# Aakash1312/Fluid-Simulation

Hardware: AMD Instinct MI355X
Metric: simulated substeps/sec (higher is better)
Workload: dtype f64

## Files before the change

### fluid-simulation_amd/csrc/common.h

```cpp
#pragma once
#include <hip/hip_runtime.h>
#include <stdint.h>

namespace fl {

constexpr uint8_t F_SOLID = 1;
constexpr uint8_t F_FLUID = 2;
constexpr int F_CNT_SHIFT = 2;

struct Grid {
    int N;
    int lo;
    int hi;
    int nx, ny, nz;
    int ox, oy, oz;
    __host__ __device__ inline size_t idx(int ix, int iy, int iz) const
    {
        return ((size_t)ix * ny + (size_t)iy) * nz + (size_t)iz;
    }
    __host__ __device__ inline size_t cells() const { return (size_t)nx * ny * nz; }
    __host__ __device__ inline long sx() const { return (long)ny * nz; }
    __host__ __device__ inline int cx0() const { return lo + ox; }
    __host__ __device__ inline int cy0() const { return lo + oy; }
    __host__ __device__ inline int cz0() const { return lo + oz; }
// ... 58 lines not shown
    int max_cell;
    int n_drop;
    int n_tl_mg, n_tl_sq;
    int n_rows, n_l1_old;
    int n_tl_int, n_tl_bnd;
    int n_l1_gal, n_drop_fail;
    unsigned long long max_speed_bits;
    double dt;
    double err_num;
    double err_den;
};

constexpr size_t STATE_PS_OFF = 256;
constexpr int MAX_PARTIALS = 8192;

__device__ __forceinline__ double spline(double x)
{
    if (x < 0) x *= -1.0;
    if (x < 0.5) return 1.5 * (4.0 * x * x * x - 4.0 * x * x + 2.0 / 3.0);
    if (x < 1.0) return 1.5 * ((-8.0 * (x * x * x) / 6.0) + 4.0 * x * x - 4.0 * x + 4.0 / 3.0);
    return 0;
}

__device__ __forceinline__ double spline_at(double p, int c, int d)
{
    double x = p - (double)c;
    if (d == 1) return spline(x);
    if (x < 0) x *= -1.0;
    if (x < 1.0) return 1.5 * ((-8.0 * (x * x * x) / 6.0) + 4.0 * x * x - 4.0 * x + 4.0 / 3.0);
    return 0;
}

template <typename T>
__device__ __forceinline__ T wave_sum(T v)
{
#pragma unroll
    for (int o = 32; o > 0; o >>= 1) v += __shfl_down(v, o, 64);
    return v;
}
template <typename T>
__device__ __forceinline__ T wave_max(T v)
{
#pragma unroll
    for (int o = 32; o > 0; o >>= 1) {
// ... 106 lines not shown
    uint32_t* pid;
    __host__ __device__ inline Particles shifted(long o) const
    {
        Particles q = *this;
        q.px += o; q.py += o; q.pz += o; q.vx += o; q.vy += o; q.vz += o; q.pid += o;
        return q;
    }
};
constexpr uint32_t PID_DEAD = 0xFFFFFFFFu;

void launch_bin_count(hipStream_t st, Grid g, long n, Particles p, int* key, int* slot, int* cell_count, int* part, StepState* ss);
void launch_bin_scatter(hipStream_t st, long n, const int* key, const int* slot, const int* cell_start, const uint32_t* pid, int* order,
                         uint32_t* spid);
void launch_bin_rank(hipStream_t st, long n_pos, long pos0, const int* key, const int* cell_start, const int* order, const uint32_t* spid,
                     int* order2);
void launch_reorder(hipStream_t st, long n, const int* order, Particles src, Particles dst, double* w = nullptr, long wstride = 0);
void launch_weights(hipStream_t st, long n, Particles p, double* w, long stride);
void launch_axpby_box(hipStream_t st, Grid g, Box box, double a, const double* x, double b, const double* y, double* out, const PcgState* gate = nullptr);
long p2g_max_items(Box box);
size_t p2g_part_doubles(Box box);
constexpr int P2G_PILED = 256;
void launch_p2g(hipStream_t st, Grid g, Box box, Particles p, const double* pw, long wstride, const int* cell_start, const uint8_t* flags,
                double* part, int* items, float* container, double* u, double* v, double* w, double* ub, double* vb, double* wb, int2* crowd_list = nullptr,
                Particles park = Particles{});
void launch_p2g_tiles(hipStream_t st, Grid g, Box box, Particles p, const double* pw, long wstride, const int* cell_start, const uint8_t* flags,
                      float* container, double* u, double* v, double* w, double* ub, double* vb, double* wb);
void launch_g2p_tiled(hipStream_t st, Grid g, Box pb, Particles p, const int* cell_start, const double* dcx, const double* dcy, const double* dcz,
                      const double* pcx, const double* pcy, const double* pcz, double blend, StepState* ss);
void launch_g2p(hipStream_t st, Grid g, long n, Particles p, const double* dcx, const double* dcy, const double* dcz, const double* pcx,
                const double* pcy, const double* pcz, double blend, StepState* ss);
void launch_advect(hipStream_t st, Grid g, long n, Particles p, const uint8_t* flags, double max_dt, double dx, StepState* ss);
void launch_advect_bin(hipStream_t st, Grid g, long n, Particles p, const uint8_t* flags, double max_dt, double dx, StepState* ss, int* key,
                       int* slot, int* cell_count, int* part);
void launch_pack_particles(hipStream_t st, long n, Particles p, double* pos_aos, double* vel_aos);
void launch_unpack_records(hipStream_t st, long n, const double* rec, Particles p, long off);
void launch_pack_records(hipStream_t st, long n, Particles p, long off, double* rec);
void launch_unpack_ids(hipStream_t st, long n, const double* pos, const double* vel, const uint32_t* ids, Particles p);
void launch_pack_ids(hipStream_t st, long n, Particles p, long off, double* pos, double* vel, uint32_t* ids);
void launch_unpack_particles(hipStream_t st, long n, const double* pos_aos, const double* vel_aos, Particles p);

// ... 222 lines not shown
```

### fluid-simulation_amd/csrc/fluid_api.hip

```cpp
#include "sim.h"
#include <algorithm>

using namespace fl;

static thread_local std::string g_err;
int fluid_fail(int code, const std::string& msg)
{
    g_err = msg;
    return code;
}
#define fail fluid_fail

Box fl::clip_dilate(const Box& b, int d, const Grid& g)
{
    Box r;
    r.x0 = b.x0 - d < 0 ? 0 : b.x0 - d;
    r.y0 = b.y0 - d < 0 ? 0 : b.y0 - d;
    r.z0 = b.z0 - d < 0 ? 0 : b.z0 - d;
    r.x1 = b.x1 + d > g.nx - 1 ? g.nx - 1 : b.x1 + d;
    r.y1 = b.y1 + d > g.ny - 1 ? g.ny - 1 : b.y1 + d;
    r.z1 = b.z1 + d > g.nz - 1 ? g.nz - 1 : b.z1 + d;
    return r;
}

// ... 33 lines not shown
        }
        p.e0.clear();
        p.e1.clear();
        p.pc.clear();
    }
}


static void free_particles(fluid_sim* s)
{
    for (Particles* p : {&s->pa, &s->pb}) {
        hipFree(p->px); hipFree(p->py); hipFree(p->pz); hipFree(p->vx); hipFree(p->vy); hipFree(p->vz); hipFree(p->pid);
        *p = Particles{};
    }
    hipFree(s->key); hipFree(s->slot); hipFree(s->order); hipFree(s->order2); hipFree(s->spid); hipFree(s->stage_pos); hipFree(s->stage_vel);
    s->order2 = nullptr; s->spid = nullptr; hipFree(s->pw);
    s->pw = nullptr;
    s->key = s->slot = s->order = nullptr;
    s->binned = false;
    s->stage_pos = s->stage_vel = nullptr;
    s->cap = 0;
}

int fl::alloc_particles(fluid_sim* s, long n)
{
    if (n <= s->cap) return FLUID_OK;
    n = (n + 1) & ~1L;
    free_particles(s);
    for (Particles* p : {&s->pa, &s->pb}) {
        HIPCHK(dalloc(&p->px, n)); HIPCHK(dalloc(&p->py, n)); HIPCHK(dalloc(&p->pz, n));
        HIPCHK(dalloc(&p->vx, n)); HIPCHK(dalloc(&p->vy, n)); HIPCHK(dalloc(&p->vz, n));
        HIPCHK(dalloc(&p->pid, n));
    }
    HIPCHK(dalloc(&s->key, n)); HIPCHK(dalloc(&s->slot, n)); HIPCHK(dalloc(&s->order, n)); HIPCHK(dalloc(&s->order2, n)); HIPCHK(dalloc(&s->spid, n));
    HIPCHK(dalloc(&s->stage_pos, 3 * n)); HIPCHK(dalloc(&s->stage_vel, 3 * n));
    HIPCHK(dalloc(&s->pw, 9 * n));
    HIPCHK(hipDeviceSynchronize());
    s->cap = n;
    return FLUID_OK;
}

int fl::grow_particles(fluid_sim* s, long need)
{
    if (need <= s->cap) return FLUID_OK;
    HIPCHK(hipStreamSynchronize(s->st));
    const long keep = s->p_off + s->np;
    Particles old = s->pa;
    s->pa = Particles{};
    const long ncap = ((need + need / 2) + 1) & ~1L;
    Particles nw{};
    HIPCHK(dalloc(&nw.px, ncap)); HIPCHK(dalloc(&nw.py, ncap)); HIPCHK(dalloc(&nw.pz, ncap));
// ... 2 lines not shown
    if (keep > 0) {
        HIPCHK(hipMemcpy(nw.px, old.px, keep * 8, hipMemcpyDeviceToDevice)); HIPCHK(hipMemcpy(nw.py, old.py, keep * 8, hipMemcpyDeviceToDevice));
        HIPCHK(hipMemcpy(nw.pz, old.pz, keep * 8, hipMemcpyDeviceToDevice)); HIPCHK(hipMemcpy(nw.vx, old.vx, keep * 8, hipMemcpyDeviceToDevice));
        HIPCHK(hipMemcpy(nw.vy, old.vy, keep * 8, hipMemcpyDeviceToDevice)); HIPCHK(hipMemcpy(nw.vz, old.vz, keep * 8, hipMemcpyDeviceToDevice));
        HIPCHK(hipMemcpy(nw.pid, old.pid, keep * 4, hipMemcpyDeviceToDevice));
    }
    hipFree(old.px); hipFree(old.py); hipFree(old.pz); hipFree(old.vx); hipFree(old.vy); hipFree(old.vz); hipFree(old.pid);
    free_particles(s);
    s->pa = nw;
    Particles* p = &s->pb;
    HIPCHK(dalloc(&p->px, ncap)); HIPCHK(dalloc(&p->py, ncap)); HIPCHK(dalloc(&p->pz, ncap));
    HIPCHK(dalloc(&p->vx, ncap)); HIPCHK(dalloc(&p->vy, ncap)); HIPCHK(dalloc(&p->vz, ncap));
    HIPCHK(dalloc(&p->pid, ncap));
    HIPCHK(dalloc(&s->key, ncap)); HIPCHK(dalloc(&s->slot, ncap)); HIPCHK(dalloc(&s->order, ncap)); HIPCHK(dalloc(&s->order2, ncap)); HIPCHK(dalloc(&s->spid, ncap));
    HIPCHK(dalloc(&s->stage_pos, 3 * ncap)); HIPCHK(dalloc(&s->stage_vel, 3 * ncap));
    HIPCHK(dalloc(&s->pw, 9 * ncap));
    HIPCHK(hipDeviceSynchronize());
    s->cap = ncap;
    return FLUID_OK;
}

extern "C" {

const char* fluid_last_error(void) { return g_err.c_str(); }
const char* fluid_version(void) { return "libfluid_hip 0.1 gfx950"; }

int fluid_default_params(fluid_params_t* p)
{
    if (!p) return fail(FLUID_ERR_ARG, "null params");
    memset(p, 0, sizeof(*p));
    p->n = 121;
// ... 340 lines not shown
    s->sort_hint = true;
    s->n_out = s->h_ss->n_out;
    s->max_cell = s->h_ss->max_cell;
    const StepState& h = *s->h_ss;
    if (h.bbox_max[0] < 0) {
        s->Pb = Box{0, 0, 0, -1, -1, -1};
    } else {
        s->Pb = Box{h.bbox_min[0], h.bbox_min[1], h.bbox_min[2], h.bbox_max[0], h.bbox_max[1], h.bbox_max[2]};
    }
    if (!box_empty(s->Pb)) {
        s->Rb = clip_dilate(s->Pb, 1, g);
        s->Sb = clip_dilate(s->Pb, 2, g);
    } else {
        s->Rb = s->Sb = s->Pb;
    }
    launch_reorder(s->st, s->np, s->order2, s->pa.shifted(s->p_off), s->pb, s->pw, s->cap);
    HIPCHK(hipGetLastError());
    std::swap(s->pa, s->pb);
    s->p_off = 0;
    prof_end(s, FLUID_PROF_SORT, tok);
    s->sorted = true;
    return FLUID_OK;
}

int fl::run_p2g(fluid_sim* s, const Box& box)
{
    const long ref_cells = s->p2g_ref_cells > 0 ? s->p2g_ref_cells : s->Rb.cells();
    const bool airy = s->last_num_active > 0 && (double)s->last_num_active < 0.3 * (double)ref_cells;
    const bool huge = (size_t)12 * sizeof(double) * (size_t)box.cells() > ((size_t)16 << 30);
    const bool piled = s->max_cell > P2G_PILED || airy;
    if (s->p2g_force ? s->p2g_force == 2 : huge) {
        s->stats.paths |= FLUID_PATH_P2G_TILES;
        launch_p2g_tiles(s->st, s->g, box, s->pa, s->pw, s->cap, s->cell_start, s->flags, s->container, s->u, s->v, s->w, s->ub, s->vb, s->wb);
        return FLUID_OK;
    }
    const bool crowd = s->p2g_force ? s->p2g_force == 3 : piled;
    if (crowd) {
        s->stats.paths |= FLUID_PATH_P2G_CROWD;
        const size_t nl = (size_t)s->cap / 16 + 64;
        if (nl > s->p2g_crowd_cap) {
            if (s->p2g_crowd) { HIPCHK(hipStreamSynchronize(s->st)); hipFree(s->p2g_crowd); s->p2g_crowd = nullptr; }
            HIPCHK(hipMalloc((void**)&s->p2g_crowd, nl * sizeof(int2)));
            s->p2g_crowd_cap = nl;
        }
    }
    const size_t need = p2g_part_doubles(box);
    if (need > s->p2g_part_cap) {
        if (s->p2g_part) { HIPCHK(hipStreamSynchronize(s->st)); hipFree(s->p2g_part); s->p2g_part = nullptr; }
        HIPCHK(hipMalloc((void**)&s->p2g_part, (need + need / 4) * sizeof(double)));
        s->p2g_part_cap = need + need / 4;
    }
    const size_t ni = 4 + 4 * (size_t)p2g_max_items(box);
    if (ni > s->p2g_items_cap) {
        if (s->p2g_items) { HIPCHK(hipStreamSynchronize(s->st)); hipFree(s->p2g_items); s->p2g_items = nullptr; }
        HIPCHK(hipMalloc((void**)&s->p2g_items, (ni + ni / 4) * sizeof(int)));
        HIPCHK(hipMemsetAsync(s->p2g_items, 0, 4 * sizeof(int), s->st));
        s->p2g_items_cap = ni + ni / 4;
    }
    launch_p2g(s->st, s->g, box, s->pa, s->pw, s->cap, s->cell_start, s->flags, s->p2g_part, s->p2g_items, s->container, s->u, s->v, s->w, s->ub,
               s->vb, s->wb, crowd ? s->p2g_crowd : nullptr, s->pb);
    return FLUID_OK;
}

static int phase_p2g(fluid_sim* s)
{
    HIPCHK(hipSetDevice(s->prm.device));
    int rc = phase_sort(s);
    if (rc) return rc;
    rc = clear_dirty(s);
    if (rc) return rc;
    memset(&s->stats, 0, sizeof(s->stats));
    s->stats.dt_in = s->dt;
    s->stats.dt_out = s->dt;
    for (int a = 0; a < 3; ++a) {
// ... 1019 lines not shown
```

### fluid-simulation_amd/csrc/fluid_dist.hip

```cpp
#include "sim.h"
#include "dist_kernels.h"

using namespace fl;
#define fail fluid_fail
int cuts_from_hist(int n, const int64_t* hist, int P, int32_t* cuts);

#define COMMCHK(expr)                                                                              \
    do {                                                                                           \
        if ((expr) != 0) return fail(FLUID_ERR_HIP, std::string("comm callback failed: ") + #expr); \
    } while (0)

namespace {

constexpr int HALO_W = 4;

struct IBox {
    int lo[3], hi[3];
};
inline bool ib_empty(const IBox& b) { return b.hi[0] <= b.lo[0] || b.hi[1] <= b.lo[1] || b.hi[2] <= b.lo[2]; }
inline IBox ib_isect(const IBox& a, const IBox& b)
{
    IBox r;
    for (int k = 0; k < 3; ++k) { r.lo[k] = std::max(a.lo[k], b.lo[k]); r.hi[k] = std::min(a.hi[k], b.hi[k]); }
    if (ib_empty(r)) for (int k = 0; k < 3; ++k) { r.lo[k] = a.lo[k]; r.hi[k] = a.lo[k]; }
// ... 320 lines not shown
    int rc;
    int tok = prof_begin(s, FLUID_PROF_SORT, (double)s->np);
    if ((rc = route_round(s))) return rc;
    {
        int ax0 = 0, ax1 = g.nx - 1;
        const bool guess = s->sort_hint && !box_empty(s->Pb);
        if (guess) { ax0 = std::max(0, s->Pb.x0 - 3); ax1 = std::min(g.nx - 1, s->Pb.x1 + 3); }
        if ((rc = sort_pass(s, ax0, ax1, d->h_cnt))) return rc;
        if (guess && s->h_ss->bbox_max[0] >= 0 && (s->h_ss->bbox_min[0] < std::min(ax0 + 2, s->Pb.x0) || s->h_ss->bbox_max[0] > std::max(ax1 - 2, s->Pb.x1))) {
            if ((rc = sort_pass(s, 0, g.nx - 1, d->h_cnt))) return rc;
        }
        s->sort_hint = true;
    }
    const long live = d->h_cnt[1];
    s->n_out = d->h_cnt[1] - d->h_cnt[0];
    launch_reorder(s->st, live, s->order2, s->pa.shifted(s->p_off), s->pb, s->pw, s->cap);
    HIPCHK(hipGetLastError());
    std::swap(s->pa, s->pb);
    s->p_off = 0;
    s->np = live;
    {
        const StepState& h = *s->h_ss;
        int* v = d->h_cnt + 64;
        const int o[3] = {g.ox, g.oy, g.oz};
        for (int a = 0; a < 3; ++a) {
            v[a] = h.bbox_max[a] < 0 ? 0x7fffffff : h.bbox_min[a] + o[a];
            v[3 + a] = h.bbox_max[a] < 0 ? 0x7fffffff : -(h.bbox_max[a] + o[a]);
        }
        v[6] = -h.max_cell;
        if (d->comm.size > 1) {
            HIPCHK(hipMemcpyAsync(d->d_cnt + 64, v, 7 * sizeof(int), hipMemcpyHostToDevice, s->st));
// ... 1530 lines not shown
```

### fluid-simulation_amd/csrc/kernels_particles.hip

```cpp
#include "common.h"

namespace fl {

struct BinAcc {
    int mn[3] = {0x7fffffff, 0x7fffffff, 0x7fffffff}, mx[3] = {-1, -1, -1};
    int nout = 0, cmax = 0;
};
__device__ __forceinline__ void bin_one(const Grid& g, long ncell, long i, double px, double py, double pz, bool dead, int* __restrict__ key,
                                        int* __restrict__ slot, int* __restrict__ cell_count, BinAcc& acc)
{
    int bx = (int)round(px) - g.cx0(), by = (int)round(py) - g.cy0(), bz = (int)round(pz) - g.cz0();
    bool in = bx >= 0 && bx < g.nx && by >= 0 && by < g.ny && bz >= 0 && bz < g.nz;
    int k = in ? (int)g.idx(bx, by, bz) : (int)ncell;
    if (dead) { k = (int)ncell + 1; in = false; }
    key[i] = k;
    {
        const int lane = threadIdx.x & 63;
        const int kp = __shfl_up(k, 1, 64);
        const bool head = lane == 0 || kp != k;
        const unsigned long long hm = __ballot(head);
        const unsigned long long below = hm & ((2ull << lane) - 1ull);
        const int start = 63 - __clzll((long long)below);
        const unsigned long long above = (lane == 63) ? 0ull : (hm >> (lane + 1)) << (lane + 1);
        const unsigned long long act = __ballot(true);
// ... 139 lines not shown
    if (act && (j + 1 == end || threadIdx.x == 255)) sAB[1] = b;
    __syncthreads();
    const int A = sAB[0], B = sAB[1];
    int rank = 0;
    for (int c0 = A; c0 < B; c0 += RANK_CH) {
        const int c1 = c0 + RANK_CH < B ? c0 + RANK_CH : B;
        if (c0 != A) __syncthreads();
        for (int t = c0 + threadIdx.x; t < c1; t += 256) sid[t - c0] = spid[t];
        __syncthreads();
        const int lo = a > c0 ? a : c0, hi = b < c1 ? b : c1;
        for (int t = lo; t < hi; ++t) rank += sid[t - c0] < mine;
    }
    if (act) order2[a + rank] = src;
}

__device__ __forceinline__ void axis_weights(double px, double py, double pz, double* __restrict__ w, long stride, long j)
{
    const double q[3] = {px, py, pz};
#pragma unroll
    for (int a = 0; a < 3; ++a) {
        const int b = (int)round(q[a]);
#pragma unroll
        for (int d = 0; d < 3; ++d) w[(a * 3 + d) * stride + j] = spline_at(q[a], b - 1 + d, d);
    }
}

__global__ __launch_bounds__(256) void k_reorder(long n, const int* __restrict__ order, Particles s, Particles d, double* __restrict__ w,
                                                 long wstride)
{
    long j = (long)blockIdx.x * 256 + threadIdx.x;
    if (j >= n) return;
    int i = order[j];
    const double px = s.px[i], py = s.py[i], pz = s.pz[i];
    d.px[j] = px; d.py[j] = py; d.pz[j] = pz;
    d.vx[j] = s.vx[i]; d.vy[j] = s.vy[i]; d.vz[j] = s.vz[i];
    d.pid[j] = s.pid[i];
    if (w) axis_weights(px, py, pz, w, wstride, j);
}

__global__ __launch_bounds__(256) void k_weights(long n, Particles p, double* __restrict__ w, long stride)
{
    long j = (long)blockIdx.x * 256 + threadIdx.x;
    if (j >= n) return;
    axis_weights(p.px[j], p.py[j], p.pz[j], w, stride, j);
}

constexpr int P2G_SLOTS = 256 * 4;
constexpr int P2G_THREADS = 192;
constexpr int P2G_CH = 384;
constexpr int P2G_SEG = P2G_CH / 8 + 1;
__device__ __forceinline__ int p2g_slot(int k) { return (k & 7) * P2G_SEG + (k >> 3); }
constexpr int P2G_LDS = 8 * P2G_SEG;
constexpr int P2G_HEAVY = 48;
constexpr int P2G_CROWD = 18;
constexpr int P2G_PIECE = 512;
constexpr int P2G_BUDGET = 8192;
constexpr int P2G_ZT = 62;

template <bool VEC, bool CROWD>
__global__ __launch_bounds__(P2G_THREADS, 3) void k_p2g_rows(Grid g, Box box, Particles p, const double* __restrict__ pw, long wstride,
                                                          const int* __restrict__ cell_start, double* __restrict__ part, long cells, int zt, const int* __restrict__ items,
                                                          Particles crowd, uint8_t* __restrict__ colflag, int ntz)
{
    __shared__ double sr[12][P2G_LDS];
    const int tid = threadIdx.x, e = tid >> 6, lane = tid & 63;
    for (int item = blockIdx.x; item < items[0]; item += gridDim.x) {
    const int4 wi = reinterpret_cast<const int4*>(items)[1 + item];
    const int rx = box.x0 - 1 + wi.x, Y0 = wi.y, Y1 = wi.z, tz0 = box.z0 + wi.w * zt;
    const int X = rx - 1 + e, zc = tz0 - 1 + lane;
    const bool colx = X >= box.x0 && X <= box.x1;
    const bool src = colx && zc >= 0 && zc < g.nz;
    const bool tgt = colx && lane >= 1 && lane <= zt && zc <= box.z1;
    const bool rowx = rx >= 0 && rx < g.nx;
    const int zlo = tz0 > 0 ? tz0 - 1 : 0, zhi = tz0 + zt < g.nz - 1 ? tz0 + zt : g.nz - 1;
    const double* swx = sr[e];
// ... 40 lines not shown
                ncz = cell_start[r1 + 1];
            }
        }
        if (je > jb) {
            const int ca_all = ca, n_all = cz - ca;
            if (CROWD && n_all >= P2G_CROWD) cz = ca;
            for (int cb = VEC ? (jb & ~1) : jb; cb < je; cb += P2G_CH) {
                const int ce = cb + P2G_CH < je ? cb + P2G_CH : je;
                if (CROWD) {
                    if (!__syncthreads_or((ca > cb ? ca : cb) < (cz < ce ? cz : ce))) continue;
                } else
                    __syncthreads();
                if (VEC) {
                    for (int j = cb + 2 * tid; j < ce; j += 2 * P2G_THREADS) {
                        const int k0 = p2g_slot(j - cb), k1 = p2g_slot(j + 1 - cb);
                        double2 t[6];
#pragma unroll
                        for (int q = 0; q < 6; ++q) t[q] = *reinterpret_cast<const double2*>(pw + q * wstride + j);
#pragma unroll
                        for (int q = 0; q < 6; ++q) { sr[q][k0] = t[q].x; sr[q][k1] = t[q].y; }
#pragma unroll
                        for (int q = 0; q < 3; ++q) t[q] = *reinterpret_cast<const double2*>(pw + (6 + q) * wstride + j);
                        t[3] = *reinterpret_cast<const double2*>(p.vx + j);
                        t[4] = *reinterpret_cast<const double2*>(p.vy + j);
                        t[5] = *reinterpret_cast<const double2*>(p.vz + j);
#pragma unroll
                        for (int q = 0; q < 6; ++q) { sr[6 + q][k0] = t[q].x; sr[6 + q][k1] = t[q].y; }
                    }
                } else {
                    for (int j = cb + tid; j < ce; j += P2G_THREADS) {
                        const int k = p2g_slot(j - cb);
#pragma unroll
                        for (int q = 0; q < 9; ++q) sr[q][k] = pw[q * wstride + j];
                        sr[9][k] = p.vx[j]; sr[10][k] = p.vy[j]; sr[11][k] = p.vz[j];
                    }
                }
                __syncthreads();
                int lo = ca > cb ? ca : cb, hi = cz < ce ? cz : ce;
                if (hi < lo) hi = lo;
                const bool heavy = !CROWD && hi - lo > P2G_HEAVY;
                if (!heavy) {
                    for (int j = lo; j < hi; ++j) {
                        const int k = p2g_slot(j - cb);
                        const double wx = swx[k];
                        const double vx = sr[9][k], vy = sr[10][k], vz = sr[11][k];
                        const double z0 = sr[6][k], z1 = sr[7][k], z2 = sr[8][k];
#pragma unroll
                        for (int a = 0; a < 3; ++a) {
                            const double xy = wx * sr[3 + a][k];
// ... 114 lines not shown
    }
    __syncthreads();
    if (!pieces) return;
    int at = s_base + inc - pieces;
    for (int w = 0; w < wv; ++w) at += s_w[w];
#pragma unroll
    for (int k = 0; k < 4; ++k) {
        const int n = first[k + 1] - first[k];
        if (n < P2G_CROWD) continue;
        for (int j = 0; j * P2G_PIECE < n; ++j) {
            const int len = n - j * P2G_PIECE < P2G_PIECE ? n - j * P2G_PIECE : P2G_PIECE;
            list[at++] = make_int2(first[k] + j * P2G_PIECE, (j << 9) | (len - 1));
        }
    }
}
__global__ __launch_bounds__(64 * PC_WAVES) void k_p2g_crowd_sum(Particles p, const double* __restrict__ pw, long wstride,
                                                                const int2* __restrict__ list, int* __restrict__ count, Particles park)
{
    __shared__ double sw[PC_WAVES][12][64];
    const int wv = threadIdx.x >> 6, lane = threadIdx.x & 63;
    const int n = lane & 15, gq = lane >> 4;
    const int total = count[0];
    double(*my)[64] = sw[wv];
    const double* ax = my[n < 9 ? n / 3 : 0];
    const double* ay = my[3 + (n < 9 ? n % 3 : 0)];
    const double* bz = my[6 + (n < 12 ? n >> 2 : 0)];
    const double* bv = my[8 + ((n & 3) ? (n & 3) : 1)];
    for (int ent = blockIdx.x * PC_WAVES + wv; ent < total; ent += gridDim.x * PC_WAVES) {
        const int2 en = list[ent];
        const int piece = en.y >> 9, lo = en.x, hi = lo + (en.y & 511) + 1, ca = lo - P2G_PIECE * piece;
        pc_d4 D = {0, 0, 0, 0};
        for (int b = lo; b < hi; b += 64) {
            const int j = b + lane;
            const bool ok = j < hi;
            double v[12];
#pragma unroll
            for (int q = 0; q < 9; ++q) v[q] = ok ? pw[q * wstride + j] : 0.0;
            v[9] = ok ? p.vx[j] : 0.0, v[10] = ok ? p.vy[j] : 0.0, v[11] = ok ? p.vz[j] : 0.0;
            __builtin_amdgcn_wave_barrier();
#pragma unroll
            for (int q = 0; q < 12; ++q) my[q][lane] = v[q];
            __builtin_amdgcn_wave_barrier();
            const int nb = hi - b < 64 ? hi - b : 64;
#pragma unroll 4
            for (int s4 = 0; s4 < 16; ++s4) {
                if (4 * s4 >= nb) break;
                const int k = 4 * s4 + gq;
                const double A = n < 9 ? ax[k] * ay[k] : 0.0;
                const double zw = bz[k], zv = zw * bv[k];
                const double B = n < 12 ? ((n & 3) ? zv : zw) : 0.0;
                D = __builtin_amdgcn_mfma_f64_16x16x4f64(A, B, D, 0, 0, 0);
            }
// ... 62 lines not shown
        const double wd = (double)wf;
        s[0] /= wd; s[1] /= wd; s[2] /= wd;
    }
    container[c] = wf;
    u[c] = s[0]; v[c] = s[1]; w[c] = s[2];
    ub[c] = s[0]; vb[c] = s[1]; wb[c] = s[2];
}

constexpr int P2GT_T = 2;
constexpr int P2GT_THREADS = P2GT_T * P2GT_T * 64;
constexpr int P2GT_CH = 512;
constexpr int P2GT_SEG = P2GT_CH / 8 + 1;
__device__ __forceinline__ int p2gt_slot(int k) { return (k & 7) * P2GT_SEG + (k >> 3); }
constexpr int P2GT_LDS = 8 * P2GT_SEG;

__global__ __launch_bounds__(P2GT_THREADS) void k_p2g_tiles(Grid g, Box box, Particles p, const double* __restrict__ pw, long wstride,
                                             const int* __restrict__ cell_start, const uint8_t* __restrict__ flags,
                                             float* __restrict__ container, double* __restrict__ u, double* __restrict__ v,
                                             double* __restrict__ w, double* __restrict__ ub, double* __restrict__ vb, double* __restrict__ wb,
                                             int zt)
{
    __shared__ double sw[9][P2GT_LDS];
    __shared__ double sv[3][P2GT_LDS];
    __shared__ int srow[(P2GT_T + 2) * (P2GT_T + 2)][2];
    const int tid = threadIdx.x, wv = tid >> 6, lane = tid & 63;
    const int ntz = (box.nz() + zt - 1) / zt, nty = (box.ny() + P2GT_T - 1) / P2GT_T;
    const int tile = blockIdx.x;
    const int tz = tile % ntz, ty = (tile / ntz) % nty, txs = tile / (ntz * nty);
    const int ntx = (box.nx() + P2GT_T - 1) / P2GT_T;
    const int tx = (txs & 1) ? ntx - 1 - (txs >> 1) : (txs >> 1);
    const int tx0 = box.x0 + tx * P2GT_T, ty0 = box.y0 + ty * P2GT_T, tz0 = box.z0 + tz * zt;
// ... 28 lines not shown
            const bool mine = src && dxi >= 0 && dxi <= 2 && dyi >= 0 && dyi <= 2;
            int ca = 0, cz = 0;
            if (mine) {
                const size_t r0 = g.idx(rx, ry, zc);
                ca = cell_start[r0];
                cz = cell_start[r0 + 1];
            }
            const double* swx = sw[dxi < 0 ? 0 : (dxi > 2 ? 2 : dxi)];
            const double* swy = sw[3 + (dyi < 0 ? 0 : (dyi > 2 ? 2 : dyi))];
            double S[3] = {0, 0, 0}, U[3] = {0, 0, 0}, V[3] = {0, 0, 0}, W[3] = {0, 0, 0};
            for (int cb = jb; cb < je; cb += P2GT_CH) {
                const int ce = cb + P2GT_CH < je ? cb + P2GT_CH : je;
                __syncthreads();
                for (int j = cb + tid; j < ce; j += P2GT_THREADS) {
                    const int k = p2gt_slot(j - cb);
#pragma unroll
                    for (int q = 0; q < 9; ++q) sw[q][k] = pw[q * wstride + j];
                    sv[0][k] = p.vx[j]; sv[1][k] = p.vy[j]; sv[2][k] = p.vz[j];
                }
                __syncthreads();
                int lo = ca > cb ? ca : cb, hi = cz < ce ? cz : ce;
                if (hi < lo) hi = lo;
                const bool heavy = hi - lo > P2G_HEAVY;
                if (!heavy) {
                    for (int j = lo; j < hi; ++j) {
                        const int k = p2gt_slot(j - cb);
                        const double a = swx[k] * swy[k];
                        const double vx = sv[0][k], vy = sv[1][k], vz = sv[2][k];
#pragma unroll
                        for (int d = 0; d < 3; ++d) {
                            const double cw = a * sw[6 + d][k];
                            S[d] += cw;
                            U[d] = U[d] + cw * vx;
// ... 357 lines not shown
    unsigned nb = nblk(n);
    if (nb > 1024) nb = 1024;
    hipLaunchKernelGGL(k_bin_count, dim3(nb), dim3(256), 0, st, g, n, p, key, slot, cell_count, part);
    hipLaunchKernelGGL(k_bin_bbox, dim3(1), dim3(256), 0, st, (const int*)part, (int)nb, ss);
}
void launch_bin_scatter(hipStream_t st, long n, const int* key, const int* slot, const int* cell_start, const uint32_t* pid, int* order,
                         uint32_t* spid)
{
    if (n > 0) hipLaunchKernelGGL(k_bin_scatter, dim3(nblk(n)), dim3(256), 0, st, n, key, slot, cell_start, pid, order, spid);
}
void launch_bin_rank(hipStream_t st, long n_pos, long pos0, const int* key, const int* cell_start, const int* order, const uint32_t* spid,
                     int* order2)
{
    if (n_pos > 0) hipLaunchKernelGGL(k_bin_rank, dim3(nblk(n_pos)), dim3(256), 0, st, n_pos, pos0, key, cell_start, order, spid, order2);
}
void launch_reorder(hipStream_t st, long n, const int* order, Particles src, Particles dst, double* w, long wstride)
{
    if (n > 0) hipLaunchKernelGGL(k_reorder, dim3(nblk(n)), dim3(256), 0, st, n, order, src, dst, w, wstride);
}
void launch_weights(hipStream_t st, long n, Particles p, double* w, long stride)
{
    if (n > 0) hipLaunchKernelGGL(k_weights, dim3(nblk(n)), dim3(256), 0, st, n, p, w, stride);
}
static void p2g_cut(const Box& box, int& ntz, int& zt, int& nseg)
{
    ntz = (box.nz() + P2G_ZT - 1) / P2G_ZT;
    zt = (box.nz() + ntz - 1) / ntz;
    nseg = 1;
    long best = -1;
    const long per = (long)(box.nx() + 2) * ntz;
    for (int k = 1; k <= box.ny(); ++k) {
        const long ys = (box.ny() + k - 1) / k, rounds = (per * k + P2G_SLOTS - 1) / P2G_SLOTS, cost = rounds * (ys + 2);
        if (best < 0 || cost < best) { best = cost; nseg = k; }
    }
}
size_t p2g_part_doubles(Box box)
{
    int ntz, zt, nseg;
    p2g_cut(box, ntz, zt, nseg);
    return (size_t)12 * box.cells() + ((size_t)3 * box.nx() * box.ny() * ntz + 7) / 8 + 8;
}
long p2g_max_items(Box box)
{
    int ntz, zt, nseg;
    p2g_cut(box, ntz, zt, nseg);
    return (long)(box.nx() + 2) * box.ny() * ntz;
}
void launch_p2g(hipStream_t st, Grid g, Box box, Particles p, const double* pw, long wstride, const int* cell_start, const uint8_t* flags,
                double* part, int* items, float* container, double* u, double* v, double* w, double* ub, double* vb, double* wb, int2* crowd_list,
                Particles park)
{
    int ntz, zt, nseg;
    p2g_cut(box, ntz, zt, nseg);
    const long cells = box.cells();
    const int budget = P2G_BUDGET;
    const unsigned nt = (unsigned)((box.nx() + 2) * nseg * ntz);
    hipLaunchKernelGGL(k_p2g_items, dim3(nblk((long)(box.nx() + 2) * nseg)), dim3(256), 0, st, g, box, cell_start, nseg, ntz, budget, items);
    const bool vec = ((((uintptr_t)pw | (uintptr_t)p.vx | (uintptr_t)p.vy | (uintptr_t)p.vz) & 15) == 0) && (wstride & 1) == 0;
    uint8_t* colflag = reinterpret_cast<uint8_t*>(part + 12 * cells);
    if (crowd_list) {
        Box sb = box;
        sb.x0 = sb.x0 > 0 ? sb.x0 - 1 : 0, sb.y0 = sb.y0 > 0 ? sb.y0 - 1 : 0, sb.z0 = sb.z0 > 0 ? sb.z0 - 1 : 0;
        sb.x1 = sb.x1 < g.nx - 1 ? sb.x1 + 1 : g.nx - 1, sb.y1 = sb.y1 < g.ny - 1 ? sb.y1 + 1 : g.ny - 1, sb.z1 = sb.z1 < g.nz - 1 ? sb.z1 + 1 : g.nz - 1;
        hipLaunchKernelGGL(k_p2g_crowd_list, dim3(nblk((long)sb.nx() * sb.ny() * ((sb.nz() + 3) / 4))), dim3(256), 0, st, g, sb, cell_start, crowd_list, items + 1);
        hipLaunchKernelGGL(k_p2g_crowd_sum, dim3(2048), dim3(64 * PC_WAVES), 0, st, p, pw, wstride, crowd_list, items + 1, park);
        if (vec) hipLaunchKernelGGL((k_p2g_rows<true, true>), dim3(nt), dim3(P2G_THREADS), 0, st, g, box, p, pw, wstride, cell_start, part, cells, zt, items, park, colflag, ntz);
        else hipLaunchKernelGGL((k_p2g_rows<false, true>), dim3(nt), dim3(P2G_THREADS), 0, st, g, box, p, pw, wstride, cell_start, part, cells, zt, items, park, colflag, ntz);
    } else if (vec) hipLaunchKernelGGL((k_p2g_rows<true, false>), dim3(nt), dim3(P2G_THREADS), 0, st, g, box, p, pw, wstride, cell_start, part, cells, zt, items, park, colflag, ntz);
    else hipLaunchKernelGGL((k_p2g_rows<false, false>), dim3(nt), dim3(P2G_THREADS), 0, st, g, box, p, pw, wstride, cell_start, part, cells, zt, items, park, colflag, ntz);
    hipLaunchKernelGGL(k_p2g_combine, dim3(nblk(cells)), dim3(256), 0, st, g, box, part, cells, flags, container, u, v, w, ub, vb, wb, items, colflag, zt, ntz);
}
void launch_p2g_tiles(hipStream_t st, Grid g, Box box, Particles p, const double* pw, long wstride, const int* cell_start, const uint8_t* flags,
                      float* container, double* u, double* v, double* w, double* ub, double* vb, double* wb)
{
    const int ntz = (box.nz() + P2G_ZT - 1) / P2G_ZT, zt = (box.nz() + ntz - 1) / ntz;
    const unsigned nt = (unsigned)(((box.nx() + P2GT_T - 1) / P2GT_T) * ((box.ny() + P2GT_T - 1) / P2GT_T) * ntz);
    hipLaunchKernelGGL(k_p2g_tiles, dim3(nt), dim3(P2GT_THREADS), 0, st, g, box, p, pw, wstride, cell_start, flags, container, u, v, w, ub, vb, wb, zt);
}
void launch_g2p_tiled(hipStream_t st, Grid g, Box pb, Particles p, const int* cell_start, const double* dcx, const double* dcy, const double* dcz,
                      const double* pcx, const double* pcy, const double* pcz, double blend, StepState* ss)
{
    if (pb.cells() <= 0) return;
    const unsigned nt = (unsigned)(((pb.nx() + G2P_TX - 1) / G2P_TX) * ((pb.ny() + G2P_TY - 1) / G2P_TY) * ((pb.nz() + G2P_TZ - 1) / G2P_TZ));
    if (pcx) hipLaunchKernelGGL(k_g2p_tiled<true>, dim3(nt), dim3(256), 0, st, g, pb, p, cell_start, dcx, dcy, dcz, pcx, pcy, pcz, blend, ss);
    else hipLaunchKernelGGL(k_g2p_tiled<false>, dim3(nt), dim3(256), 0, st, g, pb, p, cell_start, dcx, dcy, dcz, pcx, pcy, pcz, blend, ss);
}
void launch_g2p(hipStream_t st, Grid g, long n, Particles p, const double* dcx, const double* dcy, const double* dcz, const double* pcx,
                const double* pcy, const double* pcz, double blend, StepState* ss)
{
    if (n > 0) hipLaunchKernelGGL(k_g2p, dim3(nblk(n)), dim3(256), 0, st, g, n, p, dcx, dcy, dcz, pcx, pcy, pcz, blend, ss);
}
void launch_advect(hipStream_t st, Grid g, long n, Particles p, const uint8_t* flags, double max_dt, double dx, StepState* ss)
// ... 39 lines not shown
```

### fluid-simulation_amd/csrc/sim.h

```cpp
#pragma once
#include "common.h"
#include "../../include/fluid_hip.h"

#include <cmath>
#include <cstdio>
#include <cstdlib>
#include <cstring>
#include <string>
#include <utility>
#include <vector>

int fluid_fail(int code, const std::string& msg);
#define HIPCHK(expr)                                                                                              \
    do {                                                                                                          \
        hipError_t e_ = (expr);                                                                                   \
        if (e_ != hipSuccess)                                                                                     \
            return fluid_fail(FLUID_ERR_HIP, std::string(#expr) + ": " + hipGetErrorString(e_) + " @" + std::to_string(__LINE__)); \
    } while (0)
#include "snap_ring.h"

using namespace fl;

struct ProfClass {
    long launches = 0, sampled = 0;
// ... 42 lines not shown
    int *indices = nullptr, *scan_sums = nullptr, *ipart = nullptr;
    void *R = nullptr, *S[2] = {nullptr, nullptr}, *Q = nullptr, *X = nullptr, *Zmg = nullptr;
    double *pcx = nullptr, *pcy = nullptr, *pcz = nullptr;
    uint8_t* cntL = nullptr;
    LBox L{};
    size_t lmax = 0;
    double *part_bb = nullptr, *part_rr = nullptr, *part_rz[2] = {nullptr, nullptr}, *part_pq = nullptr, *part_err = nullptr;
    PcgState* ps = nullptr;
    PcgState* h_ps = nullptr;
    hipEvent_t ev_poll[2] = {nullptr, nullptr};
    long np = 0, cap = 0;
    Particles pa{}, pb{};
    int *key = nullptr, *slot = nullptr, *order = nullptr, *order2 = nullptr, *cell_count = nullptr, *cell_start = nullptr;
    uint32_t* spid = nullptr;
    double *stage_pos = nullptr, *stage_vel = nullptr;
    double* pw = nullptr;
    double* p2g_part = nullptr;
    size_t p2g_part_cap = 0;
    int2* p2g_crowd = nullptr;
    size_t p2g_crowd_cap = 0;
    int* p2g_items = nullptr;
    size_t p2g_items_cap = 0;
    int max_cell = 0;
    uint8_t* tl_flags = nullptr;
    int *tl_mg = nullptr, *tl_sq = nullptr;
    size_t tl_cap = 0;
    int n_tl_mg = 0, n_tl_sq = 0;
    int *row_flags = nullptr, *row_pos = nullptr, *row_list = nullptr;
    size_t row_cap = 0;
    int n_rows = 0;
    bool rows_on = true;
// ... 199 lines not shown
```

Baseline: 159.0.

## Compute spline weights inline in P2G instead of precomputing in reorder

Drops the 9-per-particle precomputed spline weight array that the reorder kernel wrote and the P2G kernels read back. The P2G row, crowd and tile kernels now load particle positions and evaluate the axis weights directly into shared memory. This trades global memory traffic (a write and a read of 9 doubles per particle) for extra f64 arithmetic inside P2G. It also replaces the division by six in the spline with a reciprocal multiply plus an FMA correction.

```diff
diff --git a/fluid-simulation_amd/csrc/common.h b/fluid-simulation_amd/csrc/common.h
--- a/fluid-simulation_amd/csrc/common.h
+++ b/fluid-simulation_amd/csrc/common.h
@@ -96,11 +96,19 @@
 constexpr size_t STATE_PS_OFF = 256;
 constexpr int MAX_PARTIALS = 8192;
 
+__device__ __forceinline__ double div6(double t)
+{
+    const double c = 0x1.5555555555555p-3;
+    const double q0 = t * c;
+    const double r = fma(-6.0, q0, t);
+    return fma(r, c, q0);
+}
+
 __device__ __forceinline__ double spline(double x)
 {
     if (x < 0) x *= -1.0;
     if (x < 0.5) return 1.5 * (4.0 * x * x * x - 4.0 * x * x + 2.0 / 3.0);
-    if (x < 1.0) return 1.5 * ((-8.0 * (x * x * x) / 6.0) + 4.0 * x * x - 4.0 * x + 4.0 / 3.0);
+    if (x < 1.0) return 1.5 * (div6(-8.0 * (x * x * x)) + 4.0 * x * x - 4.0 * x + 4.0 / 3.0);
     return 0;
 }
 
@@ -109,7 +117,7 @@
     double x = p - (double)c;
     if (d == 1) return spline(x);
     if (x < 0) x *= -1.0;
-    if (x < 1.0) return 1.5 * ((-8.0 * (x * x * x) / 6.0) + 4.0 * x * x - 4.0 * x + 4.0 / 3.0);
+    if (x < 1.0) return 1.5 * (div6(-8.0 * (x * x * x)) + 4.0 * x * x - 4.0 * x + 4.0 / 3.0);
     return 0;
 }
 
@@ -246,16 +254,15 @@
                          uint32_t* spid);
 void launch_bin_rank(hipStream_t st, long n_pos, long pos0, const int* key, const int* cell_start, const int* order, const uint32_t* spid,
                      int* order2);
-void launch_reorder(hipStream_t st, long n, const int* order, Particles src, Particles dst, double* w = nullptr, long wstride = 0);
-void launch_weights(hipStream_t st, long n, Particles p, double* w, long stride);
+void launch_reorder(hipStream_t st, long n, const int* order, Particles src, Particles dst);
 void launch_axpby_box(hipStream_t st, Grid g, Box box, double a, const double* x, double b, const double* y, double* out, const PcgState* gate = nullptr);
 long p2g_max_items(Box box);
 size_t p2g_part_doubles(Box box);
 constexpr int P2G_PILED = 256;
-void launch_p2g(hipStream_t st, Grid g, Box box, Particles p, const double* pw, long wstride, const int* cell_start, const uint8_t* flags,
+void launch_p2g(hipStream_t st, Grid g, Box box, Particles p, const int* cell_start, const uint8_t* flags,
                 double* part, int* items, float* container, double* u, double* v, double* w, double* ub, double* vb, double* wb, int2* crowd_list = nullptr,
                 Particles park = Particles{});
-void launch_p2g_tiles(hipStream_t st, Grid g, Box box, Particles p, const double* pw, long wstride, const int* cell_start, const uint8_t* flags,
+void launch_p2g_tiles(hipStream_t st, Grid g, Box box, Particles p, const int* cell_start, const uint8_t* flags,
                       float* container, double* u, double* v, double* w, double* ub, double* vb, double* wb);
 void launch_g2p_tiled(hipStream_t st, Grid g, Box pb, Particles p, const int* cell_start, const double* dcx, const double* dcy, const double* dcz,
                       const double* pcx, const double* pcy, const double* pcz, double blend, StepState* ss);
diff --git a/fluid-simulation_amd/csrc/fluid_api.hip b/fluid-simulation_amd/csrc/fluid_api.hip
--- a/fluid-simulation_amd/csrc/fluid_api.hip
+++ b/fluid-simulation_amd/csrc/fluid_api.hip
@@ -71,8 +71,7 @@
         *p = Particles{};
     }
     hipFree(s->key); hipFree(s->slot); hipFree(s->order); hipFree(s->order2); hipFree(s->spid); hipFree(s->stage_pos); hipFree(s->stage_vel);
-    s->order2 = nullptr; s->spid = nullptr; hipFree(s->pw);
-    s->pw = nullptr;
+    s->order2 = nullptr; s->spid = nullptr;
     s->key = s->slot = s->order = nullptr;
     s->binned = false;
     s->stage_pos = s->stage_vel = nullptr;
@@ -91,7 +90,6 @@
     }
     HIPCHK(dalloc(&s->key, n)); HIPCHK(dalloc(&s->slot, n)); HIPCHK(dalloc(&s->order, n)); HIPCHK(dalloc(&s->order2, n)); HIPCHK(dalloc(&s->spid, n));
     HIPCHK(dalloc(&s->stage_pos, 3 * n)); HIPCHK(dalloc(&s->stage_vel, 3 * n));
-    HIPCHK(dalloc(&s->pw, 9 * n));
     HIPCHK(hipDeviceSynchronize());
     s->cap = n;
     return FLUID_OK;
@@ -124,7 +122,6 @@
     HIPCHK(dalloc(&p->pid, ncap));
     HIPCHK(dalloc(&s->key, ncap)); HIPCHK(dalloc(&s->slot, ncap)); HIPCHK(dalloc(&s->order, ncap)); HIPCHK(dalloc(&s->order2, ncap)); HIPCHK(dalloc(&s->spid, ncap));
     HIPCHK(dalloc(&s->stage_pos, 3 * ncap)); HIPCHK(dalloc(&s->stage_vel, 3 * ncap));
-    HIPCHK(dalloc(&s->pw, 9 * ncap));
     HIPCHK(hipDeviceSynchronize());
     s->cap = ncap;
     return FLUID_OK;
@@ -495,7 +492,7 @@
     } else {
         s->Rb = s->Sb = s->Pb;
     }
-    launch_reorder(s->st, s->np, s->order2, s->pa.shifted(s->p_off), s->pb, s->pw, s->cap);
+    launch_reorder(s->st, s->np, s->order2, s->pa.shifted(s->p_off), s->pb);
     HIPCHK(hipGetLastError());
     std::swap(s->pa, s->pb);
     s->p_off = 0;
@@ -512,7 +509,7 @@
     const bool piled = s->max_cell > P2G_PILED || airy;
     if (s->p2g_force ? s->p2g_force == 2 : huge) {
         s->stats.paths |= FLUID_PATH_P2G_TILES;
-        launch_p2g_tiles(s->st, s->g, box, s->pa, s->pw, s->cap, s->cell_start, s->flags, s->container, s->u, s->v, s->w, s->ub, s->vb, s->wb);
+        launch_p2g_tiles(s->st, s->g, box, s->pa, s->cell_start, s->flags, s->container, s->u, s->v, s->w, s->ub, s->vb, s->wb);
         return FLUID_OK;
     }
     const bool crowd = s->p2g_force ? s->p2g_force == 3 : piled;
@@ -538,7 +535,7 @@
         HIPCHK(hipMemsetAsync(s->p2g_items, 0, 4 * sizeof(int), s->st));
         s->p2g_items_cap = ni + ni / 4;
     }
-    launch_p2g(s->st, s->g, box, s->pa, s->pw, s->cap, s->cell_start, s->flags, s->p2g_part, s->p2g_items, s->container, s->u, s->v, s->w, s->ub,
+    launch_p2g(s->st, s->g, box, s->pa, s->cell_start, s->flags, s->p2g_part, s->p2g_items, s->container, s->u, s->v, s->w, s->ub,
                s->vb, s->wb, crowd ? s->p2g_crowd : nullptr, s->pb);
     return FLUID_OK;
 }
diff --git a/fluid-simulation_amd/csrc/fluid_dist.hip b/fluid-simulation_amd/csrc/fluid_dist.hip
--- a/fluid-simulation_amd/csrc/fluid_dist.hip
+++ b/fluid-simulation_amd/csrc/fluid_dist.hip
@@ -358,7 +358,7 @@
     }
     const long live = d->h_cnt[1];
     s->n_out = d->h_cnt[1] - d->h_cnt[0];
-    launch_reorder(s->st, live, s->order2, s->pa.shifted(s->p_off), s->pb, s->pw, s->cap);
+    launch_reorder(s->st, live, s->order2, s->pa.shifted(s->p_off), s->pb);
     HIPCHK(hipGetLastError());
     std::swap(s->pa, s->pb);
     s->p_off = 0;
diff --git a/fluid-simulation_amd/csrc/kernels_particles.hip b/fluid-simulation_amd/csrc/kernels_particles.hip
--- a/fluid-simulation_amd/csrc/kernels_particles.hip
+++ b/fluid-simulation_amd/csrc/kernels_particles.hip
@@ -177,7 +177,7 @@
     if (act) order2[a + rank] = src;
 }
 
-__device__ __forceinline__ void axis_weights(double px, double py, double pz, double* __restrict__ w, long stride, long j)
+__device__ __forceinline__ void axis_weights(double px, double py, double pz, double* __restrict__ w, int stride, int j)
 {
     const double q[3] = {px, py, pz};
 #pragma unroll
@@ -188,24 +188,14 @@
     }
 }
 
-__global__ __launch_bounds__(256) void k_reorder(long n, const int* __restrict__ order, Particles s, Particles d, double* __restrict__ w,
-                                                 long wstride)
+__global__ __launch_bounds__(256) void k_reorder(long n, const int* __restrict__ order, Particles s, Particles d)
 {
     long j = (long)blockIdx.x * 256 + threadIdx.x;
     if (j >= n) return;
     int i = order[j];
-    const double px = s.px[i], py = s.py[i], pz = s.pz[i];
-    d.px[j] = px; d.py[j] = py; d.pz[j] = pz;
+    d.px[j] = s.px[i]; d.py[j] = s.py[i]; d.pz[j] = s.pz[i];
     d.vx[j] = s.vx[i]; d.vy[j] = s.vy[i]; d.vz[j] = s.vz[i];
     d.pid[j] = s.pid[i];
-    if (w) axis_weights(px, py, pz, w, wstride, j);
-}
-
-__global__ __launch_bounds__(256) void k_weights(long n, Particles p, double* __restrict__ w, long stride)
-{
-    long j = (long)blockIdx.x * 256 + threadIdx.x;
-    if (j >= n) return;
-    axis_weights(p.px[j], p.py[j], p.pz[j], w, stride, j);
 }
 
 constexpr int P2G_SLOTS = 256 * 4;
@@ -221,7 +211,7 @@
 constexpr int P2G_ZT = 62;
 
 template <bool VEC, bool CROWD>
-__global__ __launch_bounds__(P2G_THREADS, 3) void k_p2g_rows(Grid g, Box box, Particles p, const double* __restrict__ pw, long wstride,
+__global__ __launch_bounds__(P2G_THREADS, 3) void k_p2g_rows(Grid g, Box box, Particles p,
                                                           const int* __restrict__ cell_start, double* __restrict__ part, long cells, int zt, const int* __restrict__ items,
                                                           Particles crowd, uint8_t* __restrict__ colflag, int ntz)
 {
@@ -292,25 +282,21 @@
                 if (VEC) {
                     for (int j = cb + 2 * tid; j < ce; j += 2 * P2G_THREADS) {
                         const int k0 = p2g_slot(j - cb), k1 = p2g_slot(j + 1 - cb);
-                        double2 t[6];
-#pragma unroll
-                        for (int q = 0; q < 6; ++q) t[q] = *reinterpret_cast<const double2*>(pw + q * wstride + j);
-#pragma unroll
-                        for (int q = 0; q < 6; ++q) { sr[q][k0] = t[q].x; sr[q][k1] = t[q].y; }
-#pragma unroll
-                        for (int q = 0; q < 3; ++q) t[q] = *reinterpret_cast<const double2*>(pw + (6 + q) * wstride + j);
-                        t[3] = *reinterpret_cast<const double2*>(p.vx + j);
-                        t[4] = *reinterpret_cast<const double2*>(p.vy + j);
-                        t[5] = *reinterpret_cast<const double2*>(p.vz + j);
-#pragma unroll
-                        for (int q = 0; q < 6; ++q) { sr[6 + q][k0] = t[q].x; sr[6 + q][k1] = t[q].y; }
+                        const double2 x = *reinterpret_cast<const double2*>(p.px + j), y = *reinterpret_cast<const double2*>(p.py + j),
+                                      z = *reinterpret_cast<const double2*>(p.pz + j);
+                        const double2 vx = *reinterpret_cast<const double2*>(p.vx + j), vy = *reinterpret_cast<const double2*>(p.vy + j),
+                                      vz = *reinterpret_cast<const double2*>(p.vz + j);
+                        sr[9][k0] = vx.x; sr[10][k0] = vy.x; sr[11][k0] = vz.x;
+                        sr[9][k1] = vx.y; sr[10][k1] = vy.y; sr[11][k1] = vz.y;
+                        axis_weights(x.x, y.x, z.x, &sr[0][0], P2G_LDS, k0);
+                        axis_weights(x.y, y.y, z.y, &sr[0][0], P2G_LDS, k1);
                     }
                 } else {
                     for (int j = cb + tid; j < ce; j += P2G_THREADS) {
                         const int k = p2g_slot(j - cb);
-#pragma unroll
-                        for (int q = 0; q < 9; ++q) sr[q][k] = pw[q * wstride + j];
+                        const double x = p.px[j], y = p.py[j], z = p.pz[j];
                         sr[9][k] = p.vx[j]; sr[10][k] = p.vy[j]; sr[11][k] = p.vz[j];
+                        axis_weights(x, y, z, &sr[0][0], P2G_LDS, k);
                     }
                 }
                 __syncthreads();
@@ -455,7 +441,7 @@
         }
     }
 }
-__global__ __launch_bounds__(64 * PC_WAVES) void k_p2g_crowd_sum(Particles p, const double* __restrict__ pw, long wstride,
+__global__ __launch_bounds__(64 * PC_WAVES) void k_p2g_crowd_sum(Particles p,
                                                                 const int2* __restrict__ list, int* __restrict__ count, Particles park)
 {
     __shared__ double sw[PC_WAVES][12][64];
@@ -475,8 +461,9 @@
             const int j = b + lane;
             const bool ok = j < hi;
             double v[12];
-#pragma unroll
-            for (int q = 0; q < 9; ++q) v[q] = ok ? pw[q * wstride + j] : 0.0;
+            axis_weights(ok ? p.px[j] : 0.0, ok ? p.py[j] : 0.0, ok ? p.pz[j] : 0.0, v, 1, 0);
+#pragma unroll
+            for (int q = 0; q < 9; ++q) v[q] = ok ? v[q] : 0.0;
             v[9] = ok ? p.vx[j] : 0.0, v[10] = ok ? p.vy[j] : 0.0, v[11] = ok ? p.vz[j] : 0.0;
             __builtin_amdgcn_wave_barrier();
 #pragma unroll
@@ -569,7 +556,7 @@
 __device__ __forceinline__ int p2gt_slot(int k) { return (k & 7) * P2GT_SEG + (k >> 3); }
 constexpr int P2GT_LDS = 8 * P2GT_SEG;
 
-__global__ __launch_bounds__(P2GT_THREADS) void k_p2g_tiles(Grid g, Box box, Particles p, const double* __restrict__ pw, long wstride,
+__global__ __launch_bounds__(P2GT_THREADS) void k_p2g_tiles(Grid g, Box box, Particles p,
                                              const int* __restrict__ cell_start, const uint8_t* __restrict__ flags,
                                              float* __restrict__ container, double* __restrict__ u, double* __restrict__ v,
                                              double* __restrict__ w, double* __restrict__ ub, double* __restrict__ vb, double* __restrict__ wb,
@@ -628,9 +615,9 @@
                 __syncthreads();
                 for (int j = cb + tid; j < ce; j += P2GT_THREADS) {
                     const int k = p2gt_slot(j - cb);
-#pragma unroll
-                    for (int q = 0; q < 9; ++q) sw[q][k] = pw[q * wstride + j];
+                    const double x = p.px[j], y = p.py[j], z = p.pz[j];
                     sv[0][k] = p.vx[j]; sv[1][k] = p.vy[j]; sv[2][k] = p.vz[j];
+                    axis_weights(x, y, z, &sw[0][0], P2GT_LDS, k);
                 }
                 __syncthreads();
                 int lo = ca > cb ? ca : cb, hi = cz < ce ? cz : ce;
@@ -1018,13 +1005,9 @@
 {
     if (n_pos > 0) hipLaunchKernelGGL(k_bin_rank, dim3(nblk(n_pos)), dim3(256), 0, st, n_pos, pos0, key, cell_start, order, spid, order2);
 }
-void launch_reorder(hipStream_t st, long n, const int* order, Particles src, Particles dst, double* w, long wstride)
-{
-    if (n > 0) hipLaunchKernelGGL(k_reorder, dim3(nblk(n)), dim3(256), 0, st, n, order, src, dst, w, wstride);
-}
-void launch_weights(hipStream_t st, long n, Particles p, double* w, long stride)
-{
-    if (n > 0) hipLaunchKernelGGL(k_weights, dim3(nblk(n)), dim3(256), 0, st, n, p, w, stride);
+void launch_reorder(hipStream_t st, long n, const int* order, Particles src, Particles dst)
+{
+    if (n > 0) hipLaunchKernelGGL(k_reorder, dim3(nblk(n)), dim3(256), 0, st, n, order, src, dst);
 }
 static void p2g_cut(const Box& box, int& ntz, int& zt, int& nseg)
 {
@@ -1050,7 +1033,7 @@
     p2g_cut(box, ntz, zt, nseg);
     return (long)(box.nx() + 2) * box.ny() * ntz;
 }
-void launch_p2g(hipStream_t st, Grid g, Box box, Particles p, const double* pw, long wstride, const int* cell_start, const uint8_t* flags,
+void launch_p2g(hipStream_t st, Grid g, Box box, Particles p, const int* cell_start, const uint8_t* flags,
                 double* part, int* items, float* container, double* u, double* v, double* w, double* ub, double* vb, double* wb, int2* crowd_list,
                 Particles park)
 {
@@ -1060,26 +1043,26 @@
     const int budget = P2G_BUDGET;
     const unsigned nt = (unsigned)((box.nx() + 2) * nseg * ntz);
     hipLaunchKernelGGL(k_p2g_items, dim3(nblk((long)(box.nx() + 2) * nseg)), dim3(256), 0, st, g, box, cell_start, nseg, ntz, budget, items);
-    const bool vec = ((((uintptr_t)pw | (uintptr_t)p.vx | (uintptr_t)p.vy | (uintptr_t)p.vz) & 15) == 0) && (wstride & 1) == 0;
+    const bool vec = ((((uintptr_t)p.px | (uintptr_t)p.py | (uintptr_t)p.pz | (uintptr_t)p.vx | (uintptr_t)p.vy | (uintptr_t)p.vz) & 15) == 0);
     uint8_t* colflag = reinterpret_cast<uint8_t*>(part + 12 * cells);
     if (crowd_list) {
         Box sb = box;
         sb.x0 = sb.x0 > 0 ? sb.x0 - 1 : 0, sb.y0 = sb.y0 > 0 ? sb.y0 - 1 : 0, sb.z0 = sb.z0 > 0 ? sb.z0 - 1 : 0;
         sb.x1 = sb.x1 < g.nx - 1 ? sb.x1 + 1 : g.nx - 1, sb.y1 = sb.y1 < g.ny - 1 ? sb.y1 + 1 : g.ny - 1, sb.z1 = sb.z1 < g.nz - 1 ? sb.z1 + 1 : g.nz - 1;
         hipLaunchKernelGGL(k_p2g_crowd_list, dim3(nblk((long)sb.nx() * sb.ny() * ((sb.nz() + 3) / 4))), dim3(256), 0, st, g, sb, cell_start, crowd_list, items + 1);
-        hipLaunchKernelGGL(k_p2g_crowd_sum, dim3(2048), dim3(64 * PC_WAVES), 0, st, p, pw, wstride, crowd_list, items + 1, park);
-        if (vec) hipLaunchKernelGGL((k_p2g_rows<true, true>), dim3(nt), dim3(P2G_THREADS), 0, st, g, box, p, pw, wstride, cell_start, part, cells, zt, items, park, colflag, ntz);
-        else hipLaunchKernelGGL((k_p2g_rows<false, true>), dim3(nt), dim3(P2G_THREADS), 0, st, g, box, p, pw, wstride, cell_start, part, cells, zt, items, park, colflag, ntz);
-    } else if (vec) hipLaunchKernelGGL((k_p2g_rows<true, false>), dim3(nt), dim3(P2G_THREADS), 0, st, g, box, p, pw, wstride, cell_start, part, cells, zt, items, park, colflag, ntz);
-    else hipLaunchKernelGGL((k_p2g_rows<false, false>), dim3(nt), dim3(P2G_THREADS), 0, st, g, box, p, pw, wstride, cell_start, part, cells, zt, items, park, colflag, ntz);
+        hipLaunchKernelGGL(k_p2g_crowd_sum, dim3(2048), dim3(64 * PC_WAVES), 0, st, p, crowd_list, items + 1, park);
+        if (vec) hipLaunchKernelGGL((k_p2g_rows<true, true>), dim3(nt), dim3(P2G_THREADS), 0, st, g, box, p, cell_start, part, cells, zt, items, park, colflag, ntz);
+        else hipLaunchKernelGGL((k_p2g_rows<false, true>), dim3(nt), dim3(P2G_THREADS), 0, st, g, box, p, cell_start, part, cells, zt, items, park, colflag, ntz);
+    } else if (vec) hipLaunchKernelGGL((k_p2g_rows<true, false>), dim3(nt), dim3(P2G_THREADS), 0, st, g, box, p, cell_start, part, cells, zt, items, park, colflag, ntz);
+    else hipLaunchKernelGGL((k_p2g_rows<false, false>), dim3(nt), dim3(P2G_THREADS), 0, st, g, box, p, cell_start, part, cells, zt, items, park, colflag, ntz);
     hipLaunchKernelGGL(k_p2g_combine, dim3(nblk(cells)), dim3(256), 0, st, g, box, part, cells, flags, container, u, v, w, ub, vb, wb, items, colflag, zt, ntz);
 }
-void launch_p2g_tiles(hipStream_t st, Grid g, Box box, Particles p, const double* pw, long wstride, const int* cell_start, const uint8_t* flags,
+void launch_p2g_tiles(hipStream_t st, Grid g, Box box, Particles p, const int* cell_start, const uint8_t* flags,
                       float* container, double* u, double* v, double* w, double* ub, double* vb, double* wb)
 {
     const int ntz = (box.nz() + P2G_ZT - 1) / P2G_ZT, zt = (box.nz() + ntz - 1) / ntz;
     const unsigned nt = (unsigned)(((box.nx() + P2GT_T - 1) / P2GT_T) * ((box.ny() + P2GT_T - 1) / P2GT_T) * ntz);
-    hipLaunchKernelGGL(k_p2g_tiles, dim3(nt), dim3(P2GT_THREADS), 0, st, g, box, p, pw, wstride, cell_start, flags, container, u, v, w, ub, vb, wb, zt);
+    hipLaunchKernelGGL(k_p2g_tiles, dim3(nt), dim3(P2GT_THREADS), 0, st, g, box, p, cell_start, flags, container, u, v, w, ub, vb, wb, zt);
 }
 void launch_g2p_tiled(hipStream_t st, Grid g, Box pb, Particles p, const int* cell_start, const double* dcx, const double* dcy, const double* dcz,
                       const double* pcx, const double* pcy, const double* pcz, double blend, StepState* ss)
diff --git a/fluid-simulation_amd/csrc/sim.h b/fluid-simulation_amd/csrc/sim.h
--- a/fluid-simulation_amd/csrc/sim.h
+++ b/fluid-simulation_amd/csrc/sim.h
@@ -80,7 +80,6 @@
     int *key = nullptr, *slot = nullptr, *order = nullptr, *order2 = nullptr, *cell_count = nullptr, *cell_start = nullptr;
     uint32_t* spid = nullptr;
     double *stage_pos = nullptr, *stage_vel = nullptr;
-    double* pw = nullptr;
     double* p2g_part = nullptr;
     size_t p2g_part_cap = 0;
     int2* p2g_crowd = nullptr;
```

After: 159.8 (median of 6 runs). Within noise of the previous version (+0.5%).
